# nyashiki/nshogi-engine

Hardware: AMD Instinct MI355X
Metric: NN evals/sec at batch=512 (higher is better)
Workload: dtype f16m6 (f16 main term + e2m3 MX correction terms with per-32-channel E8M0 scales, f32 accumulate)

## Files before the change

nshogi-engine_amd/csrc/kernels/mfma_tile.h:

```cpp
#ifndef NSG_MFMA_TILE_H
#define NSG_MFMA_TILE_H

#include "kernels.h"

#include <atomic>
#include <type_traits>

namespace nsg {
namespace tile {

typedef float f32x4 __attribute__((ext_vector_type(4)));
typedef unsigned int u32x4 __attribute__((ext_vector_type(4)));
typedef unsigned int u32x2 __attribute__((ext_vector_type(2)));
typedef __bf16 bf16x8 __attribute__((ext_vector_type(8)));
typedef _Float16 f16x8 __attribute__((ext_vector_type(8)));

enum Mode { kConv = 0, kHeads = 1, kDense = 2 };

#ifdef NSG_COOP_SC1_STORES
constexpr bool kCoopSameXcd = false;
#else
constexpr bool kCoopSameXcd = true;
#endif
#ifdef NSG_COOP_NO_KEEP
// ... 839 lines not shown
    } else {
    constexpr int kSlabsPerTap = kSplit ? 3 : 2;
    constexpr int kSlabs = kSlabsPerTap * G::kTaps;
    auto slabOff = [](int s) constexpr {
        const int t = s / kSlabsPerTap;
        const int r = s % kSlabsPerTap;
        const int piece = kSplit ? (r == 2 ? 4 : 0) : r * 4;
        return (G::kBoards ? ((t / 3 - 1) * 10 + (t % 3 - 1) + 11) * 16 : 0) + piece * G::kPlaneStride;
    };
    constexpr bool kDeep = (NFRAG <= 2) && (kSlabs % 9 == 0);
    constexpr int kRing = kDeep ? 9 : ((kSlabs % 3 == 0) ? 3 : 2);
    constexpr int kRingA = (kDeep || (NFRAG <= 2 && kSlabs % 3 == 0)) ? 3 : 2;
    constexpr int kMfmaPerPair = (PREC == kFp32) ? 4 : 1;
    constexpr int kWMode = !kSplit ? 0 : (kDeep ? 2 : 1);
    constexpr int kWR = (NFRAG == 1) ? 18 : 6;
    constexpr int kWSets = kWMode == 0 ? kRing : (kWMode == 1 ? 3 : kWR);
    const size_t slabStride = (size_t)nft * 64;
    const u32x4* wp = A.w + (size_t)waveGroup * NFRAG * 64 + lane + (size_t)kc0 * (2 * G::kTaps) * slabStride;
    u32x4 w[kWSets][NFRAG];
    constexpr int kLead = kWMode == 0 ? ((kRing == 2) ? 2 : kRing - 1) : (kWMode == 1 ? 2 : kWR - 2);
#pragma unroll
    for (int q = 0; q < kLead; ++q)
#pragma unroll
        for (int j = 0; j < NFRAG; ++j) w[q % kWSets][j] = wp[(size_t)q * slabStride + j * 64];
    wp += (size_t)kLead * slabStride;

    NSG_STAGE_LOAD(0)
    if constexpr (G::kBoards) {
        if (zeroLds) zeroHalo<G>(smem, tid);
    }
    if constexpr (G::kBoards) __syncthreads();
    NSG_STAGE_WRITE(0)
    __syncthreads();

    NSG_STAMP(1);
    u32x4 a[kRingA][kMFw];
    constexpr bool kFlow = (kSlabs >= 9);
    constexpr int kSlotR = (kFlow && kSplit) ? kRingA : 0;
    constexpr bool kSlot = kSlotR > 0;
    static_assert(!kFlow || kSlot || kSlabs % kRingA == 0, "ring slot must carry across chunks");
    static_assert(!kSlot || (2 * G::kTaps) % kSlotR == 0, "fragment sets must carry across chunks");
    constexpr int kBarSlab = kSlot ? (kSlotR == 2 ? kSlabs - 1 : kSlabs - 3) : kSlabs - kRingA + 1;
    constexpr int kLoadSlabs = G::kItems < 6 ? G::kItems : 6;
    constexpr int kItemsPerSlab = (G::kItems + kLoadSlabs - 1) / kLoadSlabs;
    constexpr int kWriteSlab = kBarSlab - 1;
    static_assert(!kFlow || kLoadSlabs + 2 < kWriteSlab, "tile staging order");
    if constexpr (kFlow) {
#pragma unroll
        for (int q = 0; q < (kSlot ? kSlotR - 1 : kRingA - 1); ++q)
#pragma unroll
            for (int f = 0; f < kMFw; ++f)
                a[q][f] = *reinterpret_cast<const u32x4*>(smem + abase[f] + slabOff(kSlot ? 2 * q : q));
    }
    for (int kc = 0; kc < nkc; ++kc) {
        const unsigned char* abuf = smem + (kc & 1) * G::kBuf;
        const unsigned char* nbuf = smem + ((kc + 1) & 1) * G::kBuf;
        if constexpr (!kFlow) {
#pragma unroll
            for (int q = 0; q < kRingA - 1; ++q)
#pragma unroll
                for (int f = 0; f < kMFw; ++f)
                    if (q < kSlabs) a[q][f] = *reinterpret_cast<const u32x4*>(abuf + abase[f] + slabOff(q));
        }
        if constexpr (!kFlow) { NSG_STAGE_LOAD(kc + 1 < nkc ? kc + 1 : kc) }
#pragma unroll
        for (int s = 0; s < kSlabs; ++s) {
            if constexpr (kFlow) {
                if (s == kWriteSlab) { NSG_STAGE_WRITE((kc + 1) & 1) }
                if (s == kBarSlab) __syncthreads();
            }
            bool dsReads = true;
            if constexpr (kSlot) {
                const int r = s % 3, t = s / 3;
                dsReads = (r != 1);
                const int nt = (kSlotR == 2) ? (r == 0 ? t : t + 1) : t + 1;
                const bool nlo = (kSlotR == 2) ? (r == 0) : (r == 2);
                if (r != 1) {
                    const unsigned char* src = (nt < G::kTaps) ? abuf : nbuf;
                    const int off1 = slabOff(3 * (nt % G::kTaps) + (nlo ? 2 : 0));
#pragma unroll
                    for (int f = 0; f < kMFw; ++f)
                        a[(2 * nt + (nlo ? 1 : 0)) % kSlotR][f] =
                            *reinterpret_cast<const u32x4*>(src + abase[f] + off1);
                }
            } else if (s + kRingA - 1 < kSlabs) {
                const int off1 = slabOff(s + kRingA - 1);
#pragma unroll
                for (int f = 0; f < kMFw; ++f)
                    a[(s + kRingA - 1) % kRingA][f] = *reinterpret_cast<const u32x4*>(abuf + abase[f] + off1);
            } else if constexpr (kFlow) {
                const int off1 = slabOff(s + kRingA - 1 - kSlabs);
#pragma unroll
                for (int f = 0; f < kMFw; ++f)
                    a[(s + kRingA - 1) % kRingA][f] = *reinterpret_cast<const u32x4*>(nbuf + abase[f] + off1);
            }
            int wset = s % kRing;
            bool wLoads = true;
            if constexpr (kWMode == 0) {
                if constexpr (kRing >= 3) {
#pragma unroll
                    for (int j = 0; j < NFRAG; ++j) w[(s + kRing - 1) % kRing][j] = wp[j * 64];
                }
            } else {
                const int r = s % 3, t = s / 3;
                int dst = -1;
                if constexpr (kWMode == 1) {
                    wset = (r == 1) ? 1 : (t & 1) * 2;
                    if (r == 0) dst = ((t + 1) & 1) * 2;
                    if (r == 2) dst = 1;
                } else {
                    wset = (2 * t + (r == 1 ? 1 : 0)) % kWR;
                    if (r == 0) dst = (2 * t + kWR - 2) % kWR;
                    if (r == 1) dst = (2 * t + kWR - 1) % kWR;
                }
                wLoads = dst >= 0;
                if (dst >= 0) {
#pragma unroll
                    for (int j = 0; j < NFRAG; ++j) w[dst][j] = wp[j * 64];
                    wp += slabStride;
                }
            }
            if constexpr (kFlow) {
                if (s < kLoadSlabs) {
#pragma unroll
                    for (int k = s; k < G::kItems; k += kLoadSlabs)
                        st[k] = *reinterpret_cast<const u32x4*>(A.x + srcOff[k] + (size_t)(kc + 1 < nkc ? kc + 1 : kc) * 128);
                }
            }
            const int aslot = kSlot ? (2 * (s / 3) + (s % 3 == 2 ? 1 : 0)) % kSlotR : s % kRingA;
#pragma unroll
            for (int j = 0; j < NFRAG; ++j)
#pragma unroll
                for (int f = 0; f < kMFw; ++f) mfmaSlab<PREC>(acc[f][j], w[wset][j], a[aslot][f]);
            if constexpr (kWMode == 0) {
                if constexpr (kRing == 2) {
#pragma unroll
                    for (int j = 0; j < NFRAG; ++j) w[s % 2][j] = wp[j * 64];
                }
                wp += slabStride;
            }
            if constexpr (kRing >= 3) {
#pragma unroll
                for (int f = 0; f < kMFw; ++f) {
                    if (dsReads) __builtin_amdgcn_sched_group_barrier(0x100, 1, 0);
                    if (wLoads && f < NFRAG) __builtin_amdgcn_sched_group_barrier(0x020, 1, 0);
                    if (kFlow && s < kLoadSlabs && f == NFRAG) __builtin_amdgcn_sched_group_barrier(0x020, kItemsPerSlab, 0);
                    if (kFlow && s == kWriteSlab && f < G::kItems)
                        __builtin_amdgcn_sched_group_barrier(0x200, 1, 0);
                    __builtin_amdgcn_sched_group_barrier(0x008, NFRAG * kMfmaPerPair, 0);
                }
            }
            __builtin_amdgcn_sched_barrier(0);
        }
        if constexpr (kWMode == 1 && (G::kTaps & 1)) {
#pragma unroll
            for (int j = 0; j < NFRAG; ++j) w[0][j] = w[2][j];
        }
        if constexpr (!kFlow) {
            NSG_STAGE_WRITE((kc + 1) & 1)
            __syncthreads();
        }
    }
    if constexpr (kFlow) __syncthreads();
    }

#undef NSG_STAGE_LOAD
#undef NSG_COMPUTE_ABASE
#undef NSG_PIN_ACC_AGPR
#undef NSG_STAGE_WRITE
    NSG_STAMP(2);

    const int nf0 = waveGroup * NFRAG;
    const int cbase = (nf0 >> 2) * 64 + g * 16 + (nf0 & 3) * 4;
    float bv[NFRAG * 4];
#pragma unroll
    for (int i = 0; i < NFRAG * 4; ++i) bv[i] = A.bias[cbase + i];

    if constexpr (MODE == kConv && NFRAG < 4) {
#pragma unroll
        for (int f = 0; f < kMFw; ++f) {
            const int m = (fBase + f) * 16 + li;
            if (m >= G::kRows) continue;
            const size_t grow = row0 + m;
            float v[NFRAG * 4];
#pragma unroll
            for (int j = 0; j < NFRAG; ++j)
#pragma unroll
                for (int r = 0; r < 4; ++r) v[j * 4 + r] = fmaf(acc[f][j][r], A.accScale, bv[j * 4 + r]);
            if constexpr (kSplit) {
                const size_t e = grow * (size_t)A.cout * 4 + (size_t)(cbase >> 5) * 128 + (cbase & 31) * 2;
                if (hasRes) {
#pragma unroll
                    for (int j = 0; j < NFRAG; ++j) {
                        const u32x2 rh = *reinterpret_cast<const u32x2*>(A.res + e + j * 8);
                        const u32x2 rl = *reinterpret_cast<const u32x2*>(A.res + e + 64 + j * 8);
#pragma unroll
                        for (int i = 0; i < 2; ++i) {
                            v[j * 4 + 2 * i] += f16BitsToF32((uint16_t)(rh[i] & 0xffffu)) + f16BitsToF32((uint16_t)(rl[i] & 0xffffu));
                            v[j * 4 + 2 * i + 1] += f16BitsToF32((uint16_t)(rh[i] >> 16)) + f16BitsToF32((uint16_t)(rl[i] >> 16));
                        }
                    }
                }
                if (A.relu) {
#pragma unroll
                    for (int i = 0; i < NFRAG * 4; ++i) v[i] = reluF(v[i]);
                }
#pragma unroll
                for (int j = 0; j < NFRAG; ++j) {
                    u32x2 oh, ol;
#pragma unroll
                    for (int i = 0; i < 2; ++i) {
                        uint16_t h0, l0, h1, l1;
                        splitF16(v[j * 4 + 2 * i], h0, l0);
                        splitF16(v[j * 4 + 2 * i + 1], h1, l1);
                        oh[i] = (uint32_t)h0 | ((uint32_t)h1 << 16);
                        ol[i] = (uint32_t)l0 | ((uint32_t)l1 << 16);
                    }
                    *reinterpret_cast<u32x2*>(A.y + e + j * 8) = oh;
                    *reinterpret_cast<u32x2*>(A.y + e + 64 + j * 8) = ol;
                }
            } else {
                const size_t e = (grow * (size_t)A.cout + cbase) * ES;
                if (hasRes) {
#pragma unroll
                    for (int j = 0; j < NFRAG; ++j) {
                        if constexpr (PREC == kFp32) {
                            const f32x4 rr = *reinterpret_cast<const f32x4*>(A.res + e + j * 16);
#pragma unroll
                            for (int i = 0; i < 4; ++i) v[j * 4 + i] += rr[i];
                        } else {
                            const u32x2 rr = *reinterpret_cast<const u32x2*>(A.res + e + j * 8);
                            v[j * 4 + 0] += unpackLo<PREC>(rr.x); v[j * 4 + 1] += unpackHi<PREC>(rr.x);
                            v[j * 4 + 2] += unpackLo<PREC>(rr.y); v[j * 4 + 3] += unpackHi<PREC>(rr.y);
                        }
                    }
                }
                if (A.relu) {
#pragma unroll
                    for (int i = 0; i < NFRAG * 4; ++i) v[i] = reluF(v[i]);
                }
#pragma unroll
                for (int j = 0; j < NFRAG; ++j) {
                    if constexpr (PREC == kFp32) {
                        *reinterpret_cast<f32x4*>(A.y + e + j * 16) = f32x4{v[j * 4], v[j * 4 + 1], v[j * 4 + 2], v[j * 4 + 3]};
                    } else {
                        *reinterpret_cast<u32x2*>(A.y + e + j * 8) =
                            u32x2{packPair<PREC>(v[j * 4], v[j * 4 + 1]), packPair<PREC>(v[j * 4 + 2], v[j * 4 + 3])};
                    }
                }
            }
        }
        NSG_STAMP(3);
        return;
    }

#ifdef NSG_EXP_RUNTIME
    if constexpr (MODE == kConv && NFRAG == 4 && isMx(PREC)) {
        if (A.exp & 2) {
#pragma unroll
            for (int f = 0; f < kMFw; ++f)
#pragma unroll
                for (int j = 0; j < NFRAG; ++j) asm volatile("" ::"v"(acc[f][j]));
            NSG_STAMP(3);
            return;
        }
    }
#endif
    if constexpr (MODE == kConv && NFRAG == 4) {
        constexpr int kParts = KS > 1 ? KS : SS;
        constexpr int kMFe = (kMFw + kParts - 1) / kParts;
        const int fBaseE = fBase + ((KS > 1) ? (wave % KS) * kMFe : PART * kMFe);
        constexpr int kRowB = NFRAG * 16 * ES;
        constexpr int kRowS = kRowB + 16;
        constexpr int kNP = kRowB / 64;
        constexpr int kPPR = kRowB / 16;
        constexpr int kRPI = 64 / kPPR;
        constexpr int kIPF = 16 / kRPI;
        constexpr int kFragBytes = 16 * kRowS;
        constexpr int kEpiWave = G::kEpi / NWAVES / 16 * 16;
        constexpr int kRegions = (kEpiWave / kFragBytes) < 1 ? 1 : ((kEpiWave / kFragBytes) > 4 ? 4 : (kEpiWave / kFragBytes));
        static_assert(kFragBytes <= kEpiWave, "epilogue staging does not fit");
        unsigned char* ebuf = smem + wave * kEpiWave;
        const size_t rowBytes = (size_t)A.cout * ES;
        const size_t sliceOff = (size_t)waveGroup * kRowB;
        auto pieceOff = [&](int k) -> int {
            if constexpr (kSplit || kM6) return (g >> 1) * 128 + (g & 1) * 32 + (k & 1) * 16 + (k >> 1) * 64;
            else if constexpr (kM8)
                return (g >> 1) * 128 + (k < 2 ? (g & 1) * 32 + k * 16 : 64 + (k - 2) * 32 + (g & 1) * 16);
            else return g * (kRowB / 4) + k * 16;
        };
        const bool outX3 = kM8 && A.outF16x3;
        auto pieceOffX3 = [&](int k) -> int { return (g >> 1) * 128 + (g & 1) * 32 + (k & 1) * 16 + (k >> 1) * 64; };
        const int lrow = lane / kPPR;
        const int lpc = lane % kPPR;
        const unsigned laneOff = (unsigned)lrow * (unsigned)rowBytes + (unsigned)lpc * 16u;
        const size_t tileOff = (row0 + (kPerm ? (size_t)0 : (size_t)fBaseE * 16)) * rowBytes + sliceOff;
        const unsigned char* resBase = A.res + tileOff;
        unsigned char* yBase = A.y + tileOff;
        [[maybe_unused]] __amdgpu_buffer_rsrc_t resRs, yRs;
        if constexpr (COOP) {
            resRs = __builtin_amdgcn_make_buffer_rsrc(const_cast<unsigned char*>(resBase), 0, 0x7fffffff, 0x00027000);
            yRs = __builtin_amdgcn_make_buffer_rsrc(yBase, 0, 0x7fffffff, 0x00027000);
        }
        auto resLoad = [&](size_t off_) -> u32x4 {
            if constexpr (COOP) return __builtin_bit_cast(u32x4, __builtin_amdgcn_raw_buffer_load_b128(resRs, (int)off_, 0, 16));
            else return *reinterpret_cast<const u32x4*>(resBase + off_);
        };
        auto outStore = [&](size_t off_, const u32x4& v_) {
            if constexpr (COOP) __builtin_amdgcn_raw_buffer_store_b128(v_, yRs, (int)off_, 0, kCoopSameXcd ? 0 : 16);
            else *reinterpret_cast<u32x4*>(yBase + off_) = v_;
        };
        [[maybe_unused]] const unsigned permLane = (unsigned)lpc * 16u;
        const int fBasePerm = (KS > 1) ? (wave % KS) * kMFe : PART * kMFe;
        auto rowOffs = [&](int f) -> u32x4 {
            if constexpr (kPerm) return *reinterpret_cast<const u32x4*>(smem + G::kRowTabOff + ((fBasePerm + f) * 4 + lrow) * 16);
            else return u32x4{0u, 0u, 0u, 0u};
        };
        auto rowOk = [&](int f, int it, const u32x4& ro) -> bool {
            if constexpr (kPerm) return (SIZE == 2 && KS == 1 && PART * kMFe + f < EdgeRows::kMF - 1) || ro[it] != ~0u;
            else return (fBaseE + f) * 16 + it * kRPI + lrow < rowLimit;
        };
        auto rowByte = [&](int f, int it, const u32x4& ro) -> size_t {
            if constexpr (kPerm) return (size_t)(ro[it] + permLane);
            else return (size_t)(f * 16 + it * kRPI) * rowBytes + laneOff;
        };

        constexpr int kPreFrags = (RES != 1 || minWavesPerSimd<MODE, SIZE, NWAVES, NFRAG, PREC>() > 1)
                                      ? 0 : (kMFe * kIPF <= 32 ? kMFe : 32 / kIPF);
        u32x4 rpre[kPreFrags ? kPreFrags : 1][kIPF];
        if constexpr (kPreFrags > 0) {
#pragma unroll
            for (int f = 0; f < kPreFrags; ++f) {
                const u32x4 ro = rowOffs(f);
#pragma unroll
                for (int it = 0; it < kIPF; ++it) {
                    rpre[f][it] = u32x4{0u, 0u, 0u, 0u};
                    if (__builtin_expect(rowOk(f, it, ro), 1))
                        rpre[f][it] = resLoad(rowByte(f, it, ro));
                }
            }
        }

        static_assert(kRegions >= 2, "the pipelined epilogue needs two staging regions per wave");
        [[maybe_unused]] int entLi[KEEP ? kMFe : 1], entLL[KEEP ? kMFe : 1][kIPF];
        if constexpr (KEEP) {
            static_assert(kRowB == 256 && kIPF == 4, "image staging: 256-byte row slices");
            const int slice_ = waveGroup * 2 * G::kBuf;
            auto entryByte = [&](int m_) { return m_ < G::kRows ? slice_ + (34 + m_ + ((m_ * 57) >> 9)) * 16 : -1; };
            auto rowOfFrag = [&](int fg_, int r_) -> int {
                if constexpr (kPerm) {
                    int b_ = 0, y_ = 0, x_ = 0;
                    const bool ok_ = EdgeRows::square(fg_ < EdgeRows::kMF ? fg_ : 0, r_, b_, y_, x_) && fg_ < EdgeRows::kMF;
                    return ok_ ? y_ * 9 + x_ : G::kRows;
                } else {
                    return fg_ * 16 + r_;
                }
            };
#pragma unroll
            for (int f = 0; f < kMFe; ++f) {
                entLi[f] = entryByte(rowOfFrag(fBaseE + f, li));
#pragma unroll
                for (int it = 0; it < kIPF; ++it) entLL[f][it] = entryByte(rowOfFrag(fBaseE + f, it * kRPI + lrow));
            }
        }
        auto stageAt = [&](int f, int rowIsLi, int it, int piece_) -> unsigned char* {
            if constexpr (KEEP) {
                const int e_ = rowIsLi ? entLi[f] : entLL[f][it];
                return smem + (e_ < 0 ? G::kLds + lane * 16 : e_ + (piece_ >> 3) * G::kBuf + (piece_ & 7) * G::kPlaneStride);
            } else {
                return ebuf + (f % kRegions) * kFragBytes + (rowIsLi ? li : it * kRPI + lrow) * kRowS + piece_ * 16;
            }
        };
        u32x4 rpp[2][kNP];
        u32x4 tt[kIPF];
#pragma unroll
        for (int i = -1; i <= kMFe; ++i) {
            [[maybe_unused]] u32x4 roS = u32x4{0u, 0u, 0u, 0u}, roR = u32x4{0u, 0u, 0u, 0u};
            if (i >= 1) {
                const int f = i - 1;
#pragma unroll
                for (int it = 0; it < kIPF; ++it)
                    tt[it] = *reinterpret_cast<const u32x4*>(stageAt(f, 0, it, lpc));
                roS = rowOffs(f);
            }
            if (hasRes && i + 1 < kMFe) {
                const int f = i + 1;
                if (f >= kPreFrags) roR = rowOffs(f);
                const u32x4 ro = roR;
#pragma unroll
                for (int it = 0; it < kIPF; ++it) {
                    u32x4 t = u32x4{0u, 0u, 0u, 0u};
                    if (f < kPreFrags) {
                        t = rpre[f < kPreFrags ? f : 0][it];
                    } else {
                        if (__builtin_expect(rowOk(f, it, ro), 1))
                            t = resLoad(rowByte(f, it, ro));
                    }
                    *reinterpret_cast<u32x4*>(stageAt(f, 0, it, lpc)) = t;
                }
#pragma unroll
                for (int k = 0; k < kNP; ++k) {
                    const int po = (kM6 && k >= 2) ? (g >> 1) * 128 + 96 + (k - 2) * 16 : pieceOff(k);
                    rpp[f & 1][k] = *reinterpret_cast<const u32x4*>(stageAt(f, 1, 0, po / 16));
                }
            }
            if (i >= 0 && i < kMFe) {
                const int f = i;
                float v[NFRAG * 4];
#pragma unroll
                for (int j = 0; j < NFRAG; ++j)
#pragma unroll
                    for (int r = 0; r < 4; ++r) v[j * 4 + r] = fmaf(acc[f][j][r], A.accScale, bv[j * 4 + r]);
                [[maybe_unused]] unsigned char* lrowp = ebuf + (f % kRegions) * kFragBytes + li * kRowS;
                if (hasRes) {
                    const u32x4* rp = rpp[f & 1];
                    if constexpr (PREC == kFp32) {
#pragma unroll
                        for (int k = 0; k < 4; ++k)
#pragma unroll
                            for (int i = 0; i < 4; ++i) v[k * 4 + i] += __uint_as_float(rp[k][i]);
                    } else if constexpr (kSplit) {
#pragma unroll
                        for (int k = 0; k < 2; ++k)
#pragma unroll
                            for (int i = 0; i < 4; ++i) {
                                v[k * 8 + 2 * i] += f16BitsToF32((uint16_t)(rp[k][i] & 0xffffu)) +
                                                    f16BitsToF32((uint16_t)(rp[2 + k][i] & 0xffffu));
                                v[k * 8 + 2 * i + 1] += f16BitsToF32((uint16_t)(rp[k][i] >> 16)) +
                                                        f16BitsToF32((uint16_t)(rp[2 + k][i] >> 16));
                            }
                    } else if constexpr (kM6) {
                        typedef unsigned u32x6 __attribute__((ext_vector_type(6)));
                        typedef unsigned u32x16 __attribute__((ext_vector_type(16)));
                        const bool odd = (g & 1) != 0;
                        const uint32_t c0 = odd ? rp[2].w : rp[2].x, c1 = odd ? rp[3].x : rp[2].y, c2 = odd ? rp[3].y : rp[2].z;
                        const u32x6 blk = {c0, c1, c2, c0, c1, c2};
                        const float sc = __uint_as_float((rp[3].z & 0xffu) << 23);
                        u32x16 lh;
                        asm("v_cvt_scalef32_pk32_f16_fp6 %0, %1, %2" : "=&v"(lh) : "v"(blk), "v"(sc));
                        const uint32_t le[8] = {lh.s0, lh.s1, lh.s2, lh.s3, lh.s4, lh.s5, lh.s6, lh.s7};
                        const uint32_t hh[8] = {rp[0].x, rp[0].y, rp[0].z, rp[0].w, rp[1].x, rp[1].y, rp[1].z, rp[1].w};
                        typedef float f32x2r __attribute__((ext_vector_type(2)));
                        float one = 1.0f;
                        asm("" : "+v"(one));
#pragma unroll
                        for (int d = 0; d < 8; ++d) {
                            f32x2r rs;
                            asm("v_fma_mix_f32 %0, %1, %2, %3 op_sel_hi:[1,0,1]" : "=v"(rs[0]) : "v"(hh[d]), "v"(one), "v"(le[d]));
                            asm("v_fma_mix_f32 %0, %1, %2, %3 op_sel:[1,0,1] op_sel_hi:[1,0,1]" : "=v"(rs[1]) : "v"(hh[d]), "v"(one), "v"(le[d]));
                            const f32x2r sum = f32x2r{v[2 * d], v[2 * d + 1]} + rs;
                            v[2 * d] = sum[0];
                            v[2 * d + 1] = sum[1];
                        }
                    } else if constexpr (kM8) {
                        constexpr float kLoInv = 1.0f / (float)(1 << kM8LoShift);
                        typedef float f32x2 __attribute__((ext_vector_type(2)));
#pragma unroll
                        for (int d = 0; d < 4; ++d) {
                            const f32x2 l01 = __builtin_amdgcn_cvt_pk_f32_fp8((int)rp[3][d], false);
                            const f32x2 l23 = __builtin_amdgcn_cvt_pk_f32_fp8((int)rp[3][d], true);
                            const uint32_t h01 = rp[d >> 1][(d & 1) * 2], h23 = rp[d >> 1][(d & 1) * 2 + 1];
                            v[4 * d + 0] += f16BitsToF32((uint16_t)(h01 & 0xffffu)) + l01[0] * kLoInv;
                            v[4 * d + 1] += f16BitsToF32((uint16_t)(h01 >> 16)) + l01[1] * kLoInv;
                            v[4 * d + 2] += f16BitsToF32((uint16_t)(h23 & 0xffffu)) + l23[0] * kLoInv;
                            v[4 * d + 3] += f16BitsToF32((uint16_t)(h23 >> 16)) + l23[1] * kLoInv;
                        }
                    } else {
#pragma unroll
                        for (int k = 0; k < 2; ++k)
#pragma unroll
                            for (int i = 0; i < 4; ++i) {
                                v[k * 8 + 2 * i] += unpackLo<PREC>(rp[k][i]);
                                v[k * 8 + 2 * i + 1] += unpackHi<PREC>(rp[k][i]);
                            }
                    }
                }
                if (A.relu && !(kM8 || kSplit)) {
#pragma unroll
                    for (int i = 0; i < NFRAG * 4; ++i) v[i] = reluF(v[i]);
                }
                u32x4 op[kNP];
                [[maybe_unused]] const float floorV = A.relu ? 0.f : -65000.f;
                if constexpr (PREC == kFp32) {
#pragma unroll
                    for (int k = 0; k < 4; ++k)
#pragma unroll
                        for (int i = 0; i < 4; ++i) op[k][i] = __float_as_uint(v[k * 4 + i]);
                } else if constexpr (kSplit) {
#pragma unroll
                    for (int k = 0; k < 2; ++k)
#pragma unroll
                        for (int i = 0; i < 4; ++i) {
                            uint32_t h2, l2;
                            splitF16Pair(v[k * 8 + 2 * i], v[k * 8 + 2 * i + 1], floorV, h2, l2);
                            op[k][i] = h2;
                            op[2 + k][i] = l2;
                        }
                } else if constexpr (kM8) {
                    if (__builtin_expect(outX3, false)) {
#pragma unroll
                        for (int k = 0; k < 2; ++k)
#pragma unroll
                            for (int i = 0; i < 4; ++i) {
                            uint32_t h2, l2;
                            splitF16Pair(v[k * 8 + 2 * i], v[k * 8 + 2 * i + 1], floorV, h2, l2);
                            op[k][i] = h2;
                            op[2 + k][i] = l2;
                        }
                    } else if constexpr (kM6) {
                        typedef float f32x2 __attribute__((ext_vector_type(2)));
                        typedef _Float16 f16x2 __attribute__((ext_vector_type(2)));
                        typedef unsigned u32x2v __attribute__((ext_vector_type(2)));
                        typedef unsigned u32x6 __attribute__((ext_vector_type(6)));
                        typedef unsigned u32x16 __attribute__((ext_vector_type(16)));
                        typedef unsigned short u16x2 __attribute__((ext_vector_type(2)));
                        uint32_t hpv[8], sa[8], sb[8];
                        float mh = 0.f, ml = 0.f;
                        float mone = -1.0f;
                        asm("" : "+v"(mone));
                        (void)sizeof(u16x2);
#pragma unroll
                        for (int d = 0; d < 8; ++d) {
                            const f32x2 x = {__builtin_amdgcn_fmed3f(v[2 * d], floorV, 65000.f),
                                             __builtin_amdgcn_fmed3f(v[2 * d + 1], floorV, 65000.f)};
                            const f16x2 h = __builtin_convertvector(x, f16x2);
                            const uint32_t hp = __builtin_bit_cast(uint32_t, h);
                            f32x2 lx;
                            asm("v_fma_mix_f32 %0, %1, %2, %3 op_sel_hi:[1,0,0]" : "=v"(lx[0]) : "v"(hp), "v"(mone), "v"(x[0]));
                            asm("v_fma_mix_f32 %0, %1, %2, %3 op_sel:[1,0,0] op_sel_hi:[1,0,0]" : "=v"(lx[1]) : "v"(hp), "v"(mone), "v"(x[1]));
                            const uint32_t lp = __builtin_bit_cast(uint32_t, __builtin_convertvector(lx, f16x2));
                            hpv[d] = hp;
                            mh = __builtin_fmaxf(__builtin_fmaxf(__builtin_fabsf(x[0]), __builtin_fabsf(x[1])), mh);
                            ml = __builtin_fmaxf(__builtin_fmaxf(__builtin_fabsf(lx[0]), __builtin_fabsf(lx[1])), ml);
                            const u32x2v sw = __builtin_amdgcn_permlane16_swap(hp, lp, false, false);
                            sa[d] = sw.x;
                            sb[d] = sw.y;
                        }
                        const uint32_t mbits = __builtin_bit_cast(uint32_t, __builtin_convertvector(f32x2{mh, ml}, f16x2));
                        const uint32_t mhb = mbits & 0xffffu, mlb = mbits >> 16;
                        op[0] = u32x4{hpv[0], hpv[1], hpv[2], hpv[3]};
                        op[1] = u32x4{hpv[4], hpv[5], hpv[6], hpv[7]};
                        const u32x16 src = {sa[0], sa[1], sa[2], sa[3], sa[4], sa[5], sa[6], sa[7],
                                            sb[0], sb[1], sb[2], sb[3], sb[4], sb[5], sb[6], sb[7]};
                        const u32x2v mm = __builtin_amdgcn_permlane16_swap(mhb, mlb, false, false);
                        const uint32_t e5 = (mm.x > mm.y ? mm.x : mm.y) >> 10;
                        const uint32_t e8 = e5 + 110u;
                        u32x6 blk;
                        const float sc = __uint_as_float(e8 << 23);
                        asm("v_cvt_scalef32_pk32_fp6_f16 %0, %1, %2" : "=&v"(blk) : "v"(src), "v"(sc));
                        op[2] = u32x4{blk.s0, blk.s1, blk.s2, blk.s3};
                        op[3] = u32x4{blk.s4, blk.s5, e8, e8};
                    } else {
                        typedef float f32x2 __attribute__((ext_vector_type(2)));
                        typedef _Float16 f16x2 __attribute__((ext_vector_type(2)));
#pragma unroll
                        for (int d = 0; d < 4; ++d) {
                            f32x2 hf[2], lf[2];
#pragma unroll
                            for (int q = 0; q < 2; ++q) {
                                const int c = 4 * d + 2 * q;
                                const f32x2 x = {__builtin_amdgcn_fmed3f(v[c], floorV, 65000.f),
                                                 __builtin_amdgcn_fmed3f(v[c + 1], floorV, 65000.f)};
                                const f16x2 h = __builtin_convertvector(x, f16x2);
                                op[c >> 3][(c & 7) >> 1] = __builtin_bit_cast(uint32_t, h);
                                const f32x2 hx = __builtin_convertvector(h, f32x2);
                                const f32x2 lx = (x - hx) * (float)(1 << kM8LoShift);
                                hf[q] = f32x2{__builtin_amdgcn_fmed3f(hx[0], -448.f, 448.f), __builtin_amdgcn_fmed3f(hx[1], -448.f, 448.f)};
                                lf[q] = f32x2{__builtin_amdgcn_fmed3f(lx[0], -448.f, 448.f), __builtin_amdgcn_fmed3f(lx[1], -448.f, 448.f)};
                            }
                            int h8 = __builtin_amdgcn_cvt_pk_fp8_f32(hf[0][0], hf[0][1], 0, false);
                            h8 = __builtin_amdgcn_cvt_pk_fp8_f32(hf[1][0], hf[1][1], h8, true);
                            int l8 = __builtin_amdgcn_cvt_pk_fp8_f32(lf[0][0], lf[0][1], 0, false);
                            l8 = __builtin_amdgcn_cvt_pk_fp8_f32(lf[1][0], lf[1][1], l8, true);
                            op[2][d] = (uint32_t)h8;
                            op[3][d] = (uint32_t)l8;
                        }
                    }
                } else {
#pragma unroll
                    for (int k = 0; k < 2; ++k)
#pragma unroll
                        for (int i = 0; i < 4; ++i) op[k][i] = packPair<PREC>(v[k * 8 + 2 * i], v[k * 8 + 2 * i + 1]);
                }
#pragma unroll
                for (int k = 0; k < kNP; ++k) {
                    if constexpr (KEEP) *reinterpret_cast<u32x4*>(stageAt(f, 1, 0, (__builtin_expect(outX3, false) ? pieceOffX3(k) : pieceOff(k)) / 16)) = op[k];
                    else *reinterpret_cast<u32x4*>(lrowp + (__builtin_expect(outX3, false) ? pieceOffX3(k) : pieceOff(k))) = op[k];
                }
            }
            if (i >= 1) {
                const int f = i - 1;
                const u32x4 ro = roS;
#pragma unroll
                for (int it = 0; it < kIPF; ++it) {
#ifdef NSG_EXP_RUNTIME
                    asm volatile("" ::"v"(tt[it]));
                    if (__builtin_expect(rowOk(f, it, ro) && !(A.exp & 1), 1))
#else
                    if (__builtin_expect(rowOk(f, it, ro), 1))
#endif
                        outStore(rowByte(f, it, ro), tt[it]);
                }
            }
        }
#ifdef NSG_DIAG_STAMPS
        asm volatile("s_waitcnt vmcnt(0)" ::: "memory");
#endif
        NSG_STAMP(3);
        return;
    }

#pragma unroll
    for (int f = 0; f < G::kMF; ++f) {
        const int m = f * 16 + li;
        const size_t grow = row0 + m;
        const bool rowOk = G::kBoards ? (m < G::kRows) : (grow <= lastRow);
        if (!rowOk) continue;
        float v[NFRAG * 4];
#pragma unroll
        for (int j = 0; j < NFRAG; ++j)
#pragma unroll
            for (int r = 0; r < 4; ++r) v[j * 4 + r] = fmaf(acc[f][j][r], A.accScale, bv[j * 4 + r]);

        if constexpr (MODE == kHeads) {
            const int b = (int)(grow / 81);
            const int sq = (int)(grow - (size_t)b * 81);
            const int vc = A.valueChannels;
#pragma unroll
            for (int i = 0; i < NFRAG * 4; ++i) {
                const int n = cbase + i;
                if (n < vc) {
                    const float r = reluF(v[i]);
                    const size_t e = (size_t)b * A.vfeatStride + (size_t)sq * vc + n;
                    if constexpr (kSplit) {
                        const int kk = sq * vc + n;
                        uint16_t hb, lb;
                        splitF16(r, hb, lb);
                        unsigned char* row = A.vfeat + (size_t)b * A.vfeatStride * 4 + (size_t)(kk >> 5) * 128 + (kk & 31) * 2;
                        *reinterpret_cast<uint16_t*>(row) = hb;
                        *reinterpret_cast<uint16_t*>(row + 64) = lb;
                    } else if constexpr (PREC == kFp32) {
                        reinterpret_cast<float*>(A.vfeat)[e] = r;
                    } else {
                        reinterpret_cast<uint16_t*>(A.vfeat)[e] = toBits16<PREC>(r);
                    }
                } else if (n < vc + 27) {
                    A.policy[(size_t)b * 2187 + (size_t)(n - vc) * 81 + sq] = v[i];
                }
            }
        } else {
            float* out = reinterpret_cast<float*>(A.y) + (size_t)blockIdx.z * A.partStride + grow * (size_t)A.cout + cbase;
#pragma unroll
            for (int j = 0; j < NFRAG; ++j)
                *reinterpret_cast<f32x4*>(out + j * 4) =
                    f32x4{acc[f][j][0] * A.accScale, acc[f][j][1] * A.accScale, acc[f][j][2] * A.accScale, acc[f][j][3] * A.accScale};
        }
    }
}

template <int PREC, int MODE, int SIZE, int NFRAG, int NWAVES, bool HAS_RES, int MS = 1, int KS = 1, int SS = 1>
__global__ __launch_bounds__(NWAVES * 64, (minWavesPerSimd<MODE, SIZE, NWAVES, NFRAG, PREC>())) void tileKernel(
    const unsigned char* x, const u32x4* w, const unsigned char* res, unsigned char* y, const float* bias,
    int kdim, int cout, int flags , float accScale, const ArgsTail T) {
    extern __shared__ __attribute__((aligned(16))) unsigned char smem[];
    const Args A{x, w, bias, res, y, T.policy, T.vfeat, kdim, cout, T.totalRows, flags & 1, T.valueChannels,
                 T.vfeatStride, accScale, (flags >> 1) & 1, T.kSplits, T.partStride, T.stamps, flags >> 2};
    if constexpr (SS == 1) {
        tileBody<PREC, MODE, SIZE, NFRAG, NWAVES, HAS_RES ? 1 : 0, MS, KS>(A, smem, true);
    } else {
        const int part = __builtin_amdgcn_readfirstlane((int)(threadIdx.x >> 6)) % SS;
        if (part == 0) tileBody<PREC, MODE, SIZE, NFRAG, NWAVES, HAS_RES ? 1 : 0, MS, KS, SS, 0>(A, smem, true);
        else if (part == 1) tileBody<PREC, MODE, SIZE, NFRAG, NWAVES, HAS_RES ? 1 : 0, MS, KS, SS, 1>(A, smem, true);
        else if constexpr (SS > 2) {
            if (part == 2) tileBody<PREC, MODE, SIZE, NFRAG, NWAVES, HAS_RES ? 1 : 0, MS, KS, SS, 2>(A, smem, true);
            else tileBody<PREC, MODE, SIZE, NFRAG, NWAVES, HAS_RES ? 1 : 0, MS, KS, SS, 3>(A, smem, true);
        }
    }
}

template <int PREC, int SIZE, int NFRAG, int NWAVES>
__global__ __launch_bounds__(NWAVES * 64, (minWavesPerSimd<kConv, SIZE, NWAVES, NFRAG, PREC>())) void trunkKernel(
    const Args* __restrict__ layers, int nLayers, int skewTicks) {
    extern __shared__ __attribute__((aligned(16))) unsigned char smem[];
    if (skewTicks > 0) {
        const unsigned long long t0 = __builtin_amdgcn_s_memrealtime();
        const unsigned long long wait = (unsigned long long)skewTicks * ((blockIdx.x >> 3) & 7);
        while (__builtin_amdgcn_s_memrealtime() - t0 < wait) __builtin_amdgcn_s_sleep(16);
    }
    for (int l = 0; l < nLayers; ++l) {
        const Args A = layers[l];
        if (A.res) tileBody<PREC, kConv, SIZE, NFRAG, NWAVES, 1>(A, smem, true);
        else tileBody<PREC, kConv, SIZE, NFRAG, NWAVES, 0>(A, smem, true);
        __syncthreads();
    }
}

template <int PREC, int NFRAG, int NWAVES, int MS, int KS>
__global__ __launch_bounds__(NWAVES * 64, 1) void coopTrunkKernel(const Args* __restrict__ layers, int nLayers, int boards,
                                                                  unsigned* flags, unsigned flagBase, int* status, int faultBoard) {
    extern __shared__ __attribute__((aligned(16))) unsigned char smem[];
    using G = Geom<kConv, 1, NWAVES, 8>;
    if ((int)blockIdx.x >= boards) return;
    const int members = (int)(gridDim.y * gridDim.z), me = (int)(blockIdx.z * gridDim.y + blockIdx.y);
    if ((int)blockIdx.x == faultBoard && me == 1) return;
    unsigned xcc = 0;
    if constexpr (kCoopSameXcd) {
        asm volatile("s_getreg_b32 %0, hwreg(HW_REG_XCC_ID, 0, 4)" : "=s"(xcc));
        if (faultBoard == -2 && me == 1) xcc ^= 1u;
    }
    int* gaveUp = reinterpret_cast<int*>(smem + G::kLdsAlloc);
    unsigned* mine = flags + (size_t)blockIdx.x * members;
    if (threadIdx.x == 0) *gaveUp = 0;
    for (int l = 0; l < nLayers; ++l) {
        const Args A = layers[l];
        asm volatile("" ::"s"(A.x), "s"(A.w), "s"(A.res), "s"(A.y), "s"(A.bias), "s"(A.kdim), "s"(A.cout), "s"(A.relu), "s"(A.accScale),
                     "s"(A.outF16x3));
        if (l > 0) {
            if ((int)threadIdx.x < members && (int)threadIdx.x != me) {
                int spins = 0;
                unsigned seen;
                while (((seen = __hip_atomic_load(mine + threadIdx.x, __ATOMIC_RELAXED, __HIP_MEMORY_SCOPE_AGENT)) & 0xffffffu) < flagBase + (unsigned)l) {
                    if ((++spins & 255) == 0 &&
                        (spins > (1 << 21) || __hip_atomic_load(status, __ATOMIC_RELAXED, __HIP_MEMORY_SCOPE_SYSTEM) != 0)) {
                        __hip_atomic_store(status, 1, __ATOMIC_RELAXED, __HIP_MEMORY_SCOPE_SYSTEM);
                        *gaveUp = 1;
                        seen = xcc << 24;
                        break;
                    }
                    __builtin_amdgcn_s_sleep(4);
                }
                if (kCoopSameXcd && (seen >> 24) != xcc) {
                    __hip_atomic_store(status, 2, __ATOMIC_RELAXED, __HIP_MEMORY_SCOPE_SYSTEM);
                    *gaveUp = 1;
                }
            }
            __syncthreads();
            if (*gaveUp) return;
        }
        constexpr bool kKeep = kCoopKeepOwnSlice && MS == 1;
        if (A.res) tileBody<PREC, kConv, 1, NFRAG, NWAVES, 1, MS, KS, 1, 0, true, kKeep>(A, smem, true, l > 0);
        else tileBody<PREC, kConv, 1, NFRAG, NWAVES, 0, MS, KS, 1, 0, true, kKeep>(A, smem, true, l > 0);
        asm volatile("s_waitcnt vmcnt(0)" ::: "memory");
        __syncthreads();
        if (threadIdx.x == 0) __hip_atomic_store(mine + me, (flagBase + (unsigned)(l + 1)) | (xcc << 24), __ATOMIC_RELAXED, __HIP_MEMORY_SCOPE_AGENT);
    }
}

template <int PREC, int NFRAG, int NWAVES, int MS, int KS>
hipError_t launchCoopOne(const Args* layers, int nLayers, int boards, int cout, unsigned* flags, unsigned flagBase, int* status,
                         hipStream_t stream, int faultBoard) {
    using G = Geom<kConv, 1, NWAVES, 8>;
    constexpr bool kRowWG = (MS > 1 && KS > 1);
    constexpr int kChanGroups = NWAVES / (kRowWG ? KS : MS * KS);
    const int gy = cout / (kChanGroups * NFRAG * 16);
    if (gy < 1 || gy * kChanGroups * NFRAG * 16 != cout || gy * (kRowWG ? MS : 1) > 64) return hipErrorInvalidValue;
    auto k = coopTrunkKernel<PREC, NFRAG, NWAVES, MS, KS>;
    static std::atomic<int> attrDevMask{0};
    int dev = 0;
    (void)hipGetDevice(&dev);
    if (!(attrDevMask.load() & (1 << dev))) {
        const hipError_t err = hipFuncSetAttribute((const void*)k, hipFuncAttributeMaxDynamicSharedMemorySize, G::kLdsAlloc + 16);
        if (err != hipSuccess) return err;
        attrDevMask.fetch_or(1 << dev);
    }
    hipLaunchKernelGGL(k, dim3((boards + 7) / 8 * 8, gy, kRowWG ? MS : 1), dim3(G::kThreads), G::kLdsAlloc + 16, stream, layers, nLayers,
                       boards, flags, flagBase, status, faultBoard);
    return hipGetLastError();
}

#ifdef NSG_EXP_RUNTIME
inline int expFlags() { const char* e = getenv("NSG_EXP_FLAGS"); return e ? atoi(e) << 2 : 0; }
#else
constexpr int expFlags() { return 0; }
#endif

template <int PREC, int MODE, int SIZE, int NFRAG, int NWAVES, int MS = 1, int KS = 1, int SS = 1>
hipError_t launchOne(const Args& a, int gridX, hipStream_t stream) {
    using G = Geom<MODE, SIZE, NWAVES, (isMx(PREC) ? (KS > 1 ? 8 : 4) : 2)>;
    constexpr bool kRowWG = (MS > 1 && KS > 1);
    constexpr int kChanGroups = NWAVES / (kRowWG ? KS : MS * KS * SS);
    const int gy = a.cout / (kChanGroups * NFRAG * 16);
    if (gy < 1 || gy * kChanGroups * NFRAG * 16 != a.cout) return hipErrorInvalidValue;
    if (KS > 1) {
        const int chunks = a.kdim * 4 / 128;
        if (chunks > 8 || chunks % (2 * KS) != 0) return hipErrorInvalidValue;
    }
    hipError_t err;
    if (MODE == kConv && a.res) {
        auto k = tileKernel<PREC, MODE, SIZE, NFRAG, NWAVES, (MODE == kConv), MS, KS, SS>;
        static std::atomic<int> attrDevMask{0};
        int dev = 0;
        (void)hipGetDevice(&dev);
        if (!(attrDevMask.load() & (1 << dev))) {
            err = hipFuncSetAttribute((const void*)k, hipFuncAttributeMaxDynamicSharedMemorySize, G::kLdsAlloc);
            if (err != hipSuccess) return err;
            attrDevMask.fetch_or(1 << dev);
        }
        hipLaunchKernelGGL(k, dim3(gridX, gy, kRowWG ? MS : 1), dim3(G::kThreads), G::kLdsAlloc, stream, a.x, a.w, a.res, a.y, a.bias,
                           a.kdim, a.cout, (a.relu ? 1 : 0) | (a.outF16x3 ? 2 : 0) | expFlags(), a.accScale, tailOf(a));
    } else {
        auto k = tileKernel<PREC, MODE, SIZE, NFRAG, NWAVES, false, MS, KS, SS>;
        static std::atomic<int> attrDevMask{0};
        int dev = 0;
        (void)hipGetDevice(&dev);
        if (!(attrDevMask.load() & (1 << dev))) {
            err = hipFuncSetAttribute((const void*)k, hipFuncAttributeMaxDynamicSharedMemorySize, G::kLdsAlloc);
            if (err != hipSuccess) return err;
            attrDevMask.fetch_or(1 << dev);
        }
        hipLaunchKernelGGL(k, dim3(gridX, gy, MODE == kDense ? a.kSplits : (kRowWG ? MS : 1)), dim3(G::kThreads), G::kLdsAlloc, stream,
                           a.x, a.w, a.res, a.y, a.bias, a.kdim, a.cout, (a.relu ? 1 : 0) | (a.outF16x3 ? 2 : 0) | expFlags(), a.accScale, tailOf(a));
    }
    return hipGetLastError();
}

template <int PREC, int SIZE, int NFRAG, int NWAVES>
hipError_t launchTrunkOne(const Args* layers, int nLayers, int gridX, hipStream_t stream) {
    using G = Geom<kConv, SIZE, NWAVES, (isMx(PREC) ? 4 : 2)>;
    auto k = trunkKernel<PREC, SIZE, NFRAG, NWAVES>;
    hipError_t err = hipFuncSetAttribute((const void*)k, hipFuncAttributeMaxDynamicSharedMemorySize, G::kLdsAlloc);
    if (err != hipSuccess) return err;
    static const int skew = [] { const char* e = getenv("NSG_TRUNK_SKEW_US"); return e ? atoi(e) * 100 : 0; }();
    hipLaunchKernelGGL(k, dim3(gridX, 1), dim3(G::kThreads), G::kLdsAlloc, stream, layers, nLayers, skew);
    return hipGetLastError();
}

template <int PREC>
hipError_t launchTrunkPrec(const Args* layers, int nLayers, int batch, const ConvPlan& p, hipStream_t stream) {
    const int gx = (batch + p.nb - 1) / p.nb;
#define NSG_CASE(NB_, NW_) \
    if (p.nb == NB_ && p.nfrag == 4 && p.nwaves == NW_) return launchTrunkOne<PREC, NB_, 4, NW_>(layers, nLayers, gx, stream);
    NSG_CASE(2, 4) NSG_CASE(2, 3) NSG_CASE(1, 4) NSG_CASE(1, 3)
#undef NSG_CASE
    return hipErrorInvalidValue;
}
template <int PREC>
hipError_t launchConvPrec(const Args& a, int batch, const ConvPlan& p, hipStream_t stream) {
    const int gx = (batch + p.nb - 1) / p.nb;
#define NSG_CASE(NB_, NF_, NW_) \
    if (p.nb == NB_ && p.nfrag == NF_ && p.nwaves == NW_) return launchOne<PREC, kConv, NB_, NF_, NW_>(a, gx, stream);
    NSG_CASE(2, 4, 4) NSG_CASE(2, 4, 3) NSG_CASE(2, 4, 2) NSG_CASE(2, 4, 1)
    NSG_CASE(1, 4, 4) NSG_CASE(1, 4, 3) NSG_CASE(1, 4, 2) NSG_CASE(1, 4, 1)
    if (p.msplit == 2 && p.nb == 1 && p.nfrag == 2 && p.nwaves == 4) return launchOne<PREC, kConv, 1, 2, 4, 2>(a, gx, stream);
    NSG_CASE(2, 2, 4) NSG_CASE(2, 1, 4) NSG_CASE(1, 2, 4) NSG_CASE(1, 1, 4)
#undef NSG_CASE
    return hipErrorInvalidValue;
}
template <int PREC>
hipError_t launchHeadsPrec(const Args& a, hipStream_t stream) {
    constexpr int kMF = 2;
    const int gx = (a.totalRows + kMF * 16 - 1) / (kMF * 16);
    return launchOne<PREC, kHeads, kMF, 4, 1>(a, gx, stream);
}
template <int PREC>
hipError_t launchDensePrec(const Args& a, hipStream_t stream) {
    constexpr int kMF = 2;
    const int gx = (a.totalRows + kMF * 16 - 1) / (kMF * 16);
    return launchOne<PREC, kDense, kMF, 4, 1>(a, gx, stream);
}

hipError_t launchConvFp32(const Args& a, int batch, const ConvPlan& p, hipStream_t s);
hipError_t launchConvFp16(const Args& a, int batch, const ConvPlan& p, hipStream_t s);
hipError_t launchConvBf16(const Args& a, int batch, const ConvPlan& p, hipStream_t s);
hipError_t launchHeadsFp32(const Args& a, hipStream_t s);
hipError_t launchHeadsFp16(const Args& a, hipStream_t s);
hipError_t launchHeadsBf16(const Args& a, hipStream_t s);
hipError_t launchDenseFp32(const Args& a, hipStream_t s);
hipError_t launchDenseFp16(const Args& a, hipStream_t s);
hipError_t launchDenseBf16(const Args& a, hipStream_t s);
hipError_t launchConvF16x3(const Args& a, int batch, const ConvPlan& p, hipStream_t s);
hipError_t launchConvF16m8(const Args& a, int batch, const ConvPlan& p, hipStream_t s);
hipError_t launchTrunkF16m8(const Args* layers, int n, int batch, const ConvPlan& p, hipStream_t s);
hipError_t launchConvF16m6(const Args& a, int batch, const ConvPlan& p, hipStream_t s);
hipError_t launchTrunkF16m6(const Args* layers, int n, int batch, const ConvPlan& p, hipStream_t s);
hipError_t launchCoopTrunkF16m6(const Args* layers, int n, int batch, int cout, const ConvPlan& p, unsigned* flags, unsigned flagBase,
                                int* status, hipStream_t s, int faultBoard);
hipError_t launchTrunkFp32(const Args* layers, int n, int batch, const ConvPlan& p, hipStream_t s);
hipError_t launchTrunkFp16(const Args* layers, int n, int batch, const ConvPlan& p, hipStream_t s);
hipError_t launchTrunkBf16(const Args* layers, int n, int batch, const ConvPlan& p, hipStream_t s);
hipError_t launchTrunkF16x3(const Args* layers, int n, int batch, const ConvPlan& p, hipStream_t s);
hipError_t launchHeadsF16x3(const Args& a, hipStream_t s);
hipError_t launchDenseF16x3(const Args& a, hipStream_t s);

}
}

#endif
```

Measured before the change: 204,400.

## Restructure M6 epilogue: packed FMA, early hi-piece stores, global address-space residual access

Residual loads and output stores in the non-cooperative path now go through an explicit global address space pointer, so the compiler emits global rather than flat memory instructions. In the f16m6 path the accumulator scale-plus-bias becomes two-wide FMAs so packed f32 ops can be used. The fp6 decode input is built from three live words instead of a duplicated six-word vector. The encode path negates through a modifier instead of a -1 register, and stores the f16 high pieces before or after the permlane swaps depending on wave count, writing the fp6 pieces directly. The aim is to cut VALU instruction count, register pressure and flat-address overhead in the epilogue; the store-ordering split and the partial vector writes make correctness and scheduling harder to reason about.

```diff
diff --git a/nshogi-engine_amd/csrc/kernels/mfma_tile.h b/nshogi-engine_amd/csrc/kernels/mfma_tile.h
--- a/nshogi-engine_amd/csrc/kernels/mfma_tile.h
+++ b/nshogi-engine_amd/csrc/kernels/mfma_tile.h
@@ -1165,13 +1165,14 @@
             resRs = __builtin_amdgcn_make_buffer_rsrc(const_cast<unsigned char*>(resBase), 0, 0x7fffffff, 0x00027000);
             yRs = __builtin_amdgcn_make_buffer_rsrc(yBase, 0, 0x7fffffff, 0x00027000);
         }
+        typedef __attribute__((address_space(1))) u32x4 gu32x4;
         auto resLoad = [&](size_t off_) -> u32x4 {
             if constexpr (COOP) return __builtin_bit_cast(u32x4, __builtin_amdgcn_raw_buffer_load_b128(resRs, (int)off_, 0, 16));
-            else return *reinterpret_cast<const u32x4*>(resBase + off_);
+            else return *(const gu32x4*)(unsigned long long)(resBase + off_);
         };
         auto outStore = [&](size_t off_, const u32x4& v_) {
             if constexpr (COOP) __builtin_amdgcn_raw_buffer_store_b128(v_, yRs, (int)off_, 0, kCoopSameXcd ? 0 : 16);
-            else *reinterpret_cast<u32x4*>(yBase + off_) = v_;
+            else *(gu32x4*)(unsigned long long)(yBase + off_) = v_;
         };
         [[maybe_unused]] const unsigned permLane = (unsigned)lpc * 16u;
         const int fBasePerm = (KS > 1) ? (wave % KS) * kMFe : PART * kMFe;
@@ -1270,10 +1271,23 @@
             if (i >= 0 && i < kMFe) {
                 const int f = i;
                 float v[NFRAG * 4];
-#pragma unroll
-                for (int j = 0; j < NFRAG; ++j)
-#pragma unroll
-                    for (int r = 0; r < 4; ++r) v[j * 4 + r] = fmaf(acc[f][j][r], A.accScale, bv[j * 4 + r]);
+                if constexpr (kM6) {
+                    typedef float f32x2p __attribute__((ext_vector_type(2)));
+#pragma unroll
+                    for (int j = 0; j < NFRAG; ++j)
+#pragma unroll
+                        for (int r = 0; r < 4; r += 2) {
+                            const f32x2p t = __builtin_elementwise_fma(f32x2p{acc[f][j][r], acc[f][j][r + 1]}, f32x2p{A.accScale, A.accScale},
+                                                                       f32x2p{bv[j * 4 + r], bv[j * 4 + r + 1]});
+                            v[j * 4 + r] = t[0];
+                            v[j * 4 + r + 1] = t[1];
+                        }
+                } else {
+#pragma unroll
+                    for (int j = 0; j < NFRAG; ++j)
+#pragma unroll
+                        for (int r = 0; r < 4; ++r) v[j * 4 + r] = fmaf(acc[f][j][r], A.accScale, bv[j * 4 + r]);
+                }
                 [[maybe_unused]] unsigned char* lrowp = ebuf + (f % kRegions) * kFragBytes + li * kRowS;
                 if (hasRes) {
                     const u32x4* rp = rpp[f & 1];
@@ -1296,8 +1310,11 @@
                         typedef unsigned u32x6 __attribute__((ext_vector_type(6)));
                         typedef unsigned u32x16 __attribute__((ext_vector_type(16)));
                         const bool odd = (g & 1) != 0;
-                        const uint32_t c0 = odd ? rp[2].w : rp[2].x, c1 = odd ? rp[3].x : rp[2].y, c2 = odd ? rp[3].y : rp[2].z;
-                        const u32x6 blk = {c0, c1, c2, c0, c1, c2};
+                        uint32_t c0w = rp[2].w;
+                        asm("" : "+v"(c0w));
+                        const uint32_t c0 = odd ? c0w : rp[2].x, c1 = odd ? rp[3].x : rp[2].y, c2 = odd ? rp[3].y : rp[2].z;
+                        const u32x4 c012 = {c0, c1, c2, 0u};
+                        const u32x6 blk = __builtin_shufflevector(c012, c012, 0, 1, 2, -1, -1, -1);
                         const float sc = __uint_as_float((rp[3].z & 0xffu) << 23);
                         u32x16 lh;
                         asm("v_cvt_scalef32_pk32_f16_fp6 %0, %1, %2" : "=&v"(lh) : "v"(blk), "v"(sc));
@@ -1344,6 +1361,13 @@
                 }
                 u32x4 op[kNP];
                 [[maybe_unused]] const float floorV = A.relu ? 0.f : -65000.f;
+                auto pieceAddr = [&](int k) -> unsigned char* {
+                    const int po = __builtin_expect(outX3, false) ? pieceOffX3(k) : pieceOff(k);
+                    if constexpr (KEEP) return stageAt(f, 1, 0, po / 16);
+                    else return lrowp + po;
+                };
+                auto storePiece = [&](int k, const u32x4& p_) { *reinterpret_cast<u32x4*>(pieceAddr(k)) = p_; };
+                [[maybe_unused]] bool stored = false;
                 if constexpr (PREC == kFp32) {
 #pragma unroll
                     for (int k = 0; k < 4; ++k)
@@ -1377,10 +1401,10 @@
                         typedef unsigned u32x6 __attribute__((ext_vector_type(6)));
                         typedef unsigned u32x16 __attribute__((ext_vector_type(16)));
                         typedef unsigned short u16x2 __attribute__((ext_vector_type(2)));
-                        uint32_t hpv[8], sa[8], sb[8];
+                        uint32_t hpv[8], lpv[8], sa[8], sb[8];
                         float mh = 0.f, ml = 0.f;
-                        float mone = -1.0f;
-                        asm("" : "+v"(mone));
+                        float one = 1.0f;
+                        asm("" : "+v"(one));
                         (void)sizeof(u16x2);
 #pragma unroll
                         for (int d = 0; d < 8; ++d) {
@@ -1389,20 +1413,30 @@
                             const f16x2 h = __builtin_convertvector(x, f16x2);
                             const uint32_t hp = __builtin_bit_cast(uint32_t, h);
                             f32x2 lx;
-                            asm("v_fma_mix_f32 %0, %1, %2, %3 op_sel_hi:[1,0,0]" : "=v"(lx[0]) : "v"(hp), "v"(mone), "v"(x[0]));
-                            asm("v_fma_mix_f32 %0, %1, %2, %3 op_sel:[1,0,0] op_sel_hi:[1,0,0]" : "=v"(lx[1]) : "v"(hp), "v"(mone), "v"(x[1]));
-                            const uint32_t lp = __builtin_bit_cast(uint32_t, __builtin_convertvector(lx, f16x2));
+                            asm("v_fma_mix_f32 %0, -%1, %2, %3 op_sel_hi:[1,0,0]" : "=v"(lx[0]) : "v"(hp), "v"(one), "v"(x[0]));
+                            asm("v_fma_mix_f32 %0, -%1, %2, %3 op_sel:[1,0,0] op_sel_hi:[1,0,0]" : "=v"(lx[1]) : "v"(hp), "v"(one), "v"(x[1]));
                             hpv[d] = hp;
+                            lpv[d] = __builtin_bit_cast(uint32_t, __builtin_convertvector(lx, f16x2));
                             mh = __builtin_fmaxf(__builtin_fmaxf(__builtin_fabsf(x[0]), __builtin_fabsf(x[1])), mh);
                             ml = __builtin_fmaxf(__builtin_fmaxf(__builtin_fabsf(lx[0]), __builtin_fabsf(lx[1])), ml);
-                            const u32x2v sw = __builtin_amdgcn_permlane16_swap(hp, lp, false, false);
+                        }
+                        constexpr bool kHiFirst = NWAVES > 1;
+                        if constexpr (kHiFirst) {
+                            storePiece(0, u32x4{hpv[0], hpv[1], hpv[2], hpv[3]});
+                            storePiece(1, u32x4{hpv[4], hpv[5], hpv[6], hpv[7]});
+                        }
+#pragma unroll
+                        for (int d = 0; d < 8; ++d) {
+                            const u32x2v sw = __builtin_amdgcn_permlane16_swap(hpv[d], lpv[d], false, false);
                             sa[d] = sw.x;
                             sb[d] = sw.y;
                         }
+                        if constexpr (!kHiFirst) {
+                            storePiece(0, u32x4{hpv[0], hpv[1], hpv[2], hpv[3]});
+                            storePiece(1, u32x4{hpv[4], hpv[5], hpv[6], hpv[7]});
+                        }
                         const uint32_t mbits = __builtin_bit_cast(uint32_t, __builtin_convertvector(f32x2{mh, ml}, f16x2));
                         const uint32_t mhb = mbits & 0xffffu, mlb = mbits >> 16;
-                        op[0] = u32x4{hpv[0], hpv[1], hpv[2], hpv[3]};
-                        op[1] = u32x4{hpv[4], hpv[5], hpv[6], hpv[7]};
                         const u32x16 src = {sa[0], sa[1], sa[2], sa[3], sa[4], sa[5], sa[6], sa[7],
                                             sb[0], sb[1], sb[2], sb[3], sb[4], sb[5], sb[6], sb[7]};
                         const u32x2v mm = __builtin_amdgcn_permlane16_swap(mhb, mlb, false, false);
@@ -1411,8 +1445,12 @@
                         u32x6 blk;
                         const float sc = __uint_as_float(e8 << 23);
                         asm("v_cvt_scalef32_pk32_fp6_f16 %0, %1, %2" : "=&v"(blk) : "v"(src), "v"(sc));
-                        op[2] = u32x4{blk.s0, blk.s1, blk.s2, blk.s3};
-                        op[3] = u32x4{blk.s4, blk.s5, e8, e8};
+                        storePiece(2, __builtin_shufflevector(blk, blk, 0, 1, 2, 3));
+                        unsigned char* p3 = pieceAddr(3);
+                        *reinterpret_cast<u32x2v*>(p3) = __builtin_shufflevector(blk, blk, 4, 5);
+                        reinterpret_cast<uint32_t*>(p3)[2] = e8;
+                        reinterpret_cast<uint32_t*>(p3)[3] = e8;
+                        stored = true;
                     } else {
                         typedef float f32x2 __attribute__((ext_vector_type(2)));
                         typedef _Float16 f16x2 __attribute__((ext_vector_type(2)));
@@ -1445,10 +1483,9 @@
 #pragma unroll
                         for (int i = 0; i < 4; ++i) op[k][i] = packPair<PREC>(v[k * 8 + 2 * i], v[k * 8 + 2 * i + 1]);
                 }
-#pragma unroll
-                for (int k = 0; k < kNP; ++k) {
-                    if constexpr (KEEP) *reinterpret_cast<u32x4*>(stageAt(f, 1, 0, (__builtin_expect(outX3, false) ? pieceOffX3(k) : pieceOff(k)) / 16)) = op[k];
-                    else *reinterpret_cast<u32x4*>(lrowp + (__builtin_expect(outX3, false) ? pieceOffX3(k) : pieceOff(k))) = op[k];
+                if (!stored) {
+#pragma unroll
+                    for (int k = 0; k < kNP; ++k) storePiece(k, op[k]);
                 }
             }
             if (i >= 1) {
```

Result: faster. 209,800, median of 6 (+2.7%).
